# UDC-GAC/pRIblast

Measured on AMD Instinct MI355X. Metric: query RNAs/sec in `ris` step, higher is better.
Workload: dtype f64

## Files before the change

priblast_amd/csrc/capi_search.hip:

```cpp
#include <omp.h>

#include <algorithm>
#include <cmath>
#include <cstdlib>
#include <cstring>
#include <functional>

#include "search_host.hpp"

using namespace prb;

namespace prb {

struct SearchKnobs {
  double budget;
  double chunk_pairs;
  int row_shift;
  bool fused;
  bool front_ahead;
  bool sort_four_keys, sort_two_lengths;
  size_t big_list_bytes;
  int64_t gapped_chunk_hits;
  int first_tier;
  bool wave_hbm, no_resume, front_paired, front, handover;
// ... 129 lines not shown
                h.query + first, h.e_acc + first, h.e_hyb + first, h.e_tot + first};
}
static int bits_for(int64_t max_value) {
  int b = 1;
  while (b < 40 && (int64_t(1) << b) <= max_value) b++;
  return b;
}

static int sort_hits(SubSearch &s, const HitRec *recs, HitSoA out, int64_t n, const SortBounds &sb, uint32_t **perm_out) {
  prb_ctx *ctx = s.ctx;
  SearchWs &w = s.w;
  int rc;
  const size_t N = (size_t)n;
  {
    PackedKeyInfo f;
    f.qmin = sb.qmin;
    f.one_len = sb.eq_len_max > 0;
    f.lmax = f.one_len ? sb.eq_len_max : std::max(sb.max_qlen, sb.max_dblen);
    f.bl = bits_for(f.lmax);
    f.bq = bits_for(sb.max_qlen);
    f.bd = bits_for(sb.nchars);
    const int total = (f.one_len ? 1 : 2) * f.bl + f.bq + f.bd + bits_for(sb.qspan - 1);
    if (total <= 64 && f.lmax <= 65535 && !s.k.sort_four_keys) {
      if ((rc = w.kP.ensure(N * 8)) || (rc = w.kTmp2.ensure(N * 8)) || (rc = w.kE.ensure(N * 8)) || (rc = w.kTmp.ensure(N * 8)) ||
          (rc = w.idxA.ensure(N * 4)) || (rc = w.idxB.ensure(N * 4)) || (rc = w.pending.ensure(16)))
        return rc;
      PRB_HIP(launch_make_packed_keys_recs(recs, n, f, w.kP.as<uint64_t>(), w.kE.as<uint64_t>(), w.idxA.as<uint32_t>(), ctx->stream));
      if ((rc = sort_pairs(ctx->stream, w.sortTmp, w.kP.as<uint64_t>(), w.kTmp2.as<uint64_t>(), w.idxA.as<uint32_t>(),
                           w.idxB.as<uint32_t>(), N, (unsigned)total)))
        return rc;
      PRB_HIP(launch_gather_u64(w.kE.as<uint64_t>(), w.idxB.as<uint32_t>(), w.kTmp.as<uint64_t>(), n, ctx->stream));
      PRB_HIP(hipMemsetAsync(w.pending.p, 0, 4, ctx->stream));
      PRB_HIP(launch_fix_ties(w.kTmp2.as<uint64_t>(), w.kTmp.as<uint64_t>(), w.idxB.as<uint32_t>(), n, recs, w.idxA.as<uint32_t>(),
                              w.pending.as<int32_t>(), ctx->stream));
      int32_t too_long = 0;
      PRB_HIP(hipMemcpyAsync(&too_long, w.pending.p, 4, hipMemcpyDeviceToHost, ctx->stream));
      PRB_HIP(hipStreamSynchronize(ctx->stream));
      if (!too_long) {
        PRB_HIP(launch_gather_recs_to_hits(recs, w.idxA.as<uint32_t>(), out, n, ctx->stream));
        *perm_out = w.idxA.as<uint32_t>();
        return PRB_OK;
      }
    }
  }
  if (s.k.debug_mem) fprintf(stderr, "[mem] sort: the general form (%lld hits)\n", (long long)n);
  if ((rc = w.hitsTmp.ensure(hits_bytes(n)))) return rc;
  const HitSoA in = carve_hits(w.hitsTmp, n);
  PRB_HIP(launch_gather_recs_to_hits(recs, nullptr, in, n, ctx->stream));
  if ((rc = w.kE.ensure(N * 8)) || (rc = w.kL.ensure(N * 4)) || (rc = w.kQ.ensure(N * 4)) || (rc = w.kP.ensure(N * 8)) ||
      (rc = w.kTmp.ensure(N * 8)) || (rc = w.kTmp2.ensure(N * 8)) || (rc = w.idxA.ensure(N * 4)) ||
      (rc = w.idxB.ensure(N * 4)))
    return rc;
  PRB_HIP(launch_make_keys(in, n, w.kE.as<uint64_t>(), w.kL.as<uint32_t>(), w.kQ.as<uint32_t>(), w.kP.as<uint64_t>(),
                           w.idxA.as<uint32_t>(), ctx->stream));
  uint32_t *ia = w.idxA.as<uint32_t>(), *ib = w.idxB.as<uint32_t>();
  auto sort_step = [&](auto *keys, unsigned bits) -> int {
    using K = std::remove_pointer_t<decltype(keys)>;
    if (int r = sort_pairs(ctx->stream, w.sortTmp, keys, w.kTmp2.as<K>(), ia, ib, N, bits)) return r;
// ... 7 lines not shown
  if ((rc = sort_step(w.kTmp.as<uint64_t>(), 64))) return rc;
  PRB_HIP(launch_gather_u64(w.kE.as<uint64_t>(), ia, w.kTmp.as<uint64_t>(), n, ctx->stream));
  if ((rc = sort_step(w.kTmp.as<uint64_t>(), 64))) return rc;
  PRB_HIP(launch_gather_u32(w.kL.as<uint32_t>(), ia, w.kTmp.as<uint32_t>(), n, ctx->stream));
  if ((rc = sort_step(w.kTmp.as<uint32_t>(), 32))) return rc;
  PRB_HIP(launch_gather_u32(w.kQ.as<uint32_t>(), ia, w.kTmp.as<uint32_t>(), n, ctx->stream));
  if ((rc = sort_step(w.kTmp.as<uint32_t>(), 32))) return rc;
  PRB_HIP(launch_gather_u64(w.kP.as<uint64_t>(), ia, w.kTmp.as<uint64_t>(), n, ctx->stream));
  unsigned qbits = 1;
  while ((1 << qbits) < s.qb->nq && qbits < 31) qbits++;
  if ((rc = sort_step(w.kTmp.as<uint64_t>(), 32 + qbits))) return rc;
  PRB_HIP(launch_gather_hits(in, ia, out, n, ctx->stream));
  *perm_out = ia;
  return PRB_OK;
}

struct ToI64 {
  __host__ __device__ int64_t operator()(const int32_t &v) const { return (int64_t)v; }
};
struct MaxOp {
  __host__ __device__ int64_t operator()(const int64_t &a, const int64_t &b) const { return a > b ? a : b; }
};

static int filter_hits(prb_ctx *ctx, SearchWs &w, const HitSoA &h, int64_t n, double thr, int64_t *nsurv) {
  int rc;
  const size_t N = (size_t)n;
  *nsurv = 0;
  if (n == 0) return PRB_OK;
  if ((rc = w.endKey.ensure(N * 8)) || (rc = w.pmax.ensure(N * 8)) || (rc = w.state.ensure(N)) || (rc = w.keep.ensure(N)) ||
      (rc = w.pending.ensure(16)) || (rc = w.surv.ensure(N * 4)) || (rc = w.count.ensure(16)))
    return rc;
  PRB_HIP(launch_filter_init(h, n, thr, w.endKey.as<int64_t>(), w.state.as<uint8_t>(), ctx->stream));
  if ((rc = with_temp(w.scanTmp, "rocprim::inclusive_scan", [&](void *t, size_t &b) {
         return rocprim::inclusive_scan(t, b, w.endKey.as<int64_t>(), w.pmax.as<int64_t>(), N, MaxOp(), ctx->stream);
       })))
    return rc;
  for (int round = 0;; round++) {
    PRB_HIP(hipMemsetAsync(w.pending.p, 0, 4, ctx->stream));
    PRB_HIP(launch_filter_round(h, n, w.pmax.as<int64_t>(), w.state.as<uint8_t>(), w.pending.as<int32_t>(), ctx->stream));
    int32_t pend = 0;
    PRB_HIP(hipMemcpyAsync(&pend, w.pending.p, 4, hipMemcpyDeviceToHost, ctx->stream));
    PRB_HIP(hipStreamSynchronize(ctx->stream));
    if (!pend) break;
    if (round > 100000) {
      set_error("redundancy filter did not converge");
      return PRB_ERR_STATE;
    }
  }
  PRB_HIP(launch_filter_final(h, n, w.pmax.as<int64_t>(), w.state.as<uint8_t>(), w.keep.as<uint8_t>(), ctx->stream));
  return select_flagged(ctx, w, nullptr, w.keep.as<uint8_t>(), w.surv.as<uint32_t>(), N, nsurv);
}

static void mem_note(const char *where, const SearchWs &w) {
  static const bool on = getenv("PRB_DEBUG_MEM") != nullptr;
  if (!on) return;
  size_t free_b = 0, total_b = 0;
  (void)hipMemGetInfo(&free_b, &total_b);
  fprintf(stderr, "[mem] %-18s free %7zu MiB | hitsA %6zu hitsB %6zu hitsC %6zu hitsTmp %6zu MiB\n", where, free_b >> 20, w.hitsA.cap >> 20,
          w.hitsB.cap >> 20, w.hitsC.cap >> 20, w.hitsTmp.cap >> 20);
}

static int grow_keep(prb_ctx *ctx, DevBuf &buf, size_t have, size_t need, size_t spare_limit = SIZE_MAX) {
  int rc;
  if (have > 0 && need > buf.cap) {
    DevBuf bigger;
    if ((rc = need > spare_limit ? PRB_ERR_NOMEM : bigger.ensure(need + need / 2)) && (rc = bigger.ensure(need + need / 6)) &&
        (rc = bigger.ensure(need)))
      return rc;
    PRB_HIP(hipMemcpyAsync(bigger.p, buf.p, have, hipMemcpyDeviceToDevice, ctx->stream));
    PRB_HIP(hipStreamSynchronize(ctx->stream));
    buf.release();
    buf = bigger;
// ... 254 lines not shown
  if (big_list) {
    w.trim_next = true;
    PRB_HIP(hipStreamSynchronize(ctx->stream));
    w.front.release();
    for (DevBuf *b : {&w.hitsA, &w.hitsTmp, &w.row_count, &w.row_off, &w.row_cand, &w.seed_qacc, &w.cands, &w.trace, &w.resumePool,
                      &w.resumePool2, &w.resumePool3, &w.keptU, &w.keptTrace})
      b->release();
    for (DevBuf *b : {&ctx->ra_band, &ctx->ra_vec, &ctx->ra_codes, &ctx->ra_desc}) b->release();
    if ((rc = w.front.init())) return rc;
  }
  mem_note("before the sort", w);
  if ((rc = w.hitsC.ensure(hits_bytes(s.nf)))) return rc;
  HitSoA B = carve_hits(w.hitsC, s.nf);
  uint32_t *perm = nullptr;
  if ((rc = ctx->time_begin())) return rc;
  SortBounds sb1 = s.sb;
  if (s.all_one_pass && s.one_pass_maxlen > 0 && !s.k.sort_two_lengths) sb1.eq_len_max = (int32_t)s.one_pass_maxlen;
  if ((rc = sort_hits(s, w.hitsB.as<HitRec>(), B, s.nf, sb1, &perm))) return rc;
  if ((rc = ctx->time_end("sort", 9))) return rc;
  if (big_list)
    for (DevBuf *b : {&w.hitsB, &w.kE, &w.kL, &w.kQ, &w.kP, &w.kTmp, &w.kTmp2, &w.idxA, &w.idxB, &w.sortTmp}) b->release();
  mem_note("sorted", w);
  if ((rc = ctx->time_begin())) return rc;
  if ((rc = filter_hits(ctx, w, B, s.nf, s.opts.interaction_threshold, &s.nung))) return rc;
  if ((rc = ctx->time_end("filter", 3))) return rc;
  s.hs->counts[1] += s.nung;
  if (s.nung == 0) return PRB_OK;
  if ((rc = w.hitsA.ensure(hits_bytes(s.nung)))) return rc;
  s.U = carve_hits(w.hitsA, s.nung);
  PRB_HIP(launch_gather_hits(B, w.surv.as<uint32_t>(), s.U, s.nung, ctx->stream));
  if ((rc = w.first.ensure((size_t)s.nung))) return rc;
  PRB_HIP(launch_mark_first(s.U.query, s.nung, w.first.as<uint8_t>(), ctx->stream));
  s.first = w.first.as<uint8_t>();
  return PRB_OK;
}

static int emit_ungapped(SubSearch &s) {
  prb_hitset *hs = s.hs;
  const size_t base = hs->hits.size();
  if (int rc = download_hits(s.ctx, s.w, s.U, s.nung, hs->hits)) return rc;
  auto code_base = [](unsigned c) { return c <= 5 ? (int)c - 1 : (int)c - 5; };
  for (size_t i = base; i < hs->hits.size(); i++) {
    prb_hit &h = hs->hits[i];
    const uint8_t *qs = s.qb->enc.data() + s.qb->off[h.query];
    h.bp_offset = (int64_t)hs->bp.size() / 2;
    const int len = (int)(uint16_t)h.q_len;
    for (int j = 0; j < len; j++)
      if (s.ctx->params.bp_pair[code_base(qs[h.q_sp + j])][code_base(s.pg.seqs[h.db_sp + j])] != 0) {
// ... 310 lines not shown
  s.tier_all = w.keptTier.as<uint8_t>();
  s.ntrace_all = w.keptNtrace.as<int32_t>();
  s.trace_all = w.keptTrace.as<uint16_t>();
  return PRB_OK;
}

static int final_sort_filter(SubSearch &s) {
  prb_ctx *ctx = s.ctx;
  SearchWs &w = s.w;
  int rc;
  if (!s.chunked) {
    if ((rc = ctx->time_begin())) return rc;
    if ((rc = compact_below(ctx, w, s.G, s.nung, s.opts.final_threshold, w.cidx, w.hitsB, &s.ngap))) return rc;
    if ((rc = ctx->time_end("filter", 2))) return rc;
  }
  if (s.ngap == 0) return PRB_OK;
  if ((rc = w.hitsC.ensure(hits_bytes(s.ngap)))) return rc;
  HitSoA S = carve_hits(w.hitsC, s.ngap);
  uint32_t *perm = nullptr;
  if ((rc = ctx->time_begin())) return rc;
  if ((rc = sort_hits(s, w.hitsB.as<HitRec>(), S, s.ngap, s.sb, &perm))) return rc;
  if ((rc = ctx->time_end("sort", 9))) return rc;
  if ((rc = ctx->time_begin())) return rc;
  if ((rc = filter_hits(ctx, w, S, s.ngap, s.opts.final_threshold, &s.nfin))) return rc;
  if ((rc = ctx->time_end("filter", 3))) return rc;
  s.hs->counts[2] += s.nfin;
  if (s.nfin == 0) return PRB_OK;
  if ((rc = w.hitsB.ensure(hits_bytes(s.nfin)))) return rc;
  s.F = carve_hits(w.hitsB, s.nfin);
  PRB_HIP(launch_gather_hits(S, w.surv.as<uint32_t>(), s.F, s.nfin, ctx->stream));
  if ((rc = w.subset2.ensure((size_t)s.nfin * 4)) || (rc = w.subset.ensure((size_t)s.nfin * 4))) return rc;
  PRB_HIP(launch_gather_u32(perm, w.surv.as<uint32_t>(), w.subset2.as<uint32_t>(), s.nfin, ctx->stream));
  PRB_HIP(launch_gather_u32(w.cidx.as<uint32_t>(), w.subset2.as<uint32_t>(), w.subset.as<uint32_t>(), s.nfin, ctx->stream));
  return PRB_OK;
}

static int traceback(SubSearch &s) {
  prb_ctx *ctx = s.ctx;
  SearchWs &w = s.w;
  const int64_t nfin = s.nfin;
  const size_t NF = (size_t)nfin;
  int rc;
  if ((rc = w.copy_init())) return rc;
  if (w.copy_pending) {
    PRB_HIP(hipStreamWaitEvent(ctx->stream, w.copy_done, 0));
    w.copy_pending = false;
  }
  if ((rc = ctx->time_begin())) return rc;
// ... 560 lines not shown
```

priblast_amd/csrc/search_host.hpp:

```cpp
#pragma once
#include <atomic>
#include <chrono>
#include <condition_variable>
#include <cstring>
#include <deque>
#include <memory>
#include <mutex>
#include <thread>

#include <rocprim/rocprim.hpp>

#include "../../include/priblast_hip.h"
#include "context.hpp"
#include "db_format.hpp"
#include "hitset.hpp"
#include "output.hpp"
#include "search_kernels.hpp"
#include "seed_dfs.hpp"

namespace prb {

struct SearchConstMem {
  DevBuf ints, bulge;
  SearchConst view{};
// ... 49 lines not shown
        (void)hipStreamDestroy(stream);
        (void)hipEventDestroy(done);
        stream = nullptr;
      }
      for (DevBuf *b : {&cands, &seed_qacc, &pair0, &keyA, &keyB, &valA, &valB, &sortTmp}) b->release();
      pair0_pin.release();
      ahead = false;
    }
  } front;
  hipStream_t copy_stream = nullptr;
  hipEvent_t packed_ready = nullptr, copy_done = nullptr;
  bool copy_pending = false;
  int copy_init() {
    if (copy_stream) return PRB_OK;
    if (hipStreamCreateWithFlags(&copy_stream, hipStreamNonBlocking) != hipSuccess ||
        hipEventCreateWithFlags(&packed_ready, hipEventDisableTiming) != hipSuccess ||
        hipEventCreateWithFlags(&copy_done, hipEventDisableTiming) != hipSuccess) {
      set_error("hipStreamCreate / hipEventCreate failed (result copies)");
      return PRB_ERR_HIP;
    }
    return PRB_OK;
  }
  PinnedBuf pinned, cand_pinned[2], tb_pinned, pin_hits[2], pin_bp[2];
  bool trim_next = false;
  void trim() {
#define X(name, trimmable) \
  if (trimmable && name.cap > ((size_t)256 << 20)) name.release();
    PRB_SEARCH_BUFFERS(X)
#undef X
    trim_next = false;
  }
  void release() {
#define X(name, trimmable) name.release();
    PRB_SEARCH_BUFFERS(X)
#undef X
    front.release();
    if (copy_stream) {
      (void)hipStreamSynchronize(copy_stream);
      (void)hipStreamDestroy(copy_stream);
      (void)hipEventDestroy(packed_ready);
      (void)hipEventDestroy(copy_done);
      copy_stream = nullptr;
    }
    for (PinnedBuf *b : {&pinned, &cand_pinned[0], &cand_pinned[1], &tb_pinned, &pin_hits[0], &pin_hits[1], &pin_bp[0], &pin_bp[1]})
      b->release();
  }
};

inline SearchWs &ws_of(prb_ctx *ctx) {
  if (!ctx->search_ws) ctx->search_ws = new SearchWs();
  return *static_cast<SearchWs *>(ctx->search_ws);
}

struct Drainer {
  struct Job {
    int slot;
    int64_t nhits, nbp_ints;
  };
  std::vector<prb_hit> *hits;
  std::vector<int32_t> *bp;
  std::vector<prb_pair_summary> *pairs = nullptr;
  PinnedBuf *pin_hits, *pin_bp;
  hipEvent_t ev[2] = {nullptr, nullptr};
  std::thread th;
  std::mutex m;
  std::condition_variable cv;
  std::deque<Job> jobs;
// ... 265 lines not shown
```

priblast_amd/csrc/search_kernels.hip:

```cpp
#include "search_kernels.hpp"

#include <cstdlib>

#include "../../include/priblast_hip.h"

#include "search_device.hpp"

namespace prb {

namespace {

constexpr int kBlock = 256;

__device__ __forceinline__ int seq_of(const PageDev &pg, int sp) {
  int lo = 0, hi = pg.nseq - 1;
  while (lo < hi) {
    int m = (lo + hi + 1) >> 1;
    if (pg.start_pos[m] <= sp) lo = m;
    else hi = m - 1;
  }
  return lo;
}

__device__ __forceinline__ double window_acc(const float *acc, const float *cond, int64_t sp, int length, int delta) {
// ... 590 lines not shown
  k_energy[i] = (eb >> 63) ? ~eb : (eb | 0x8000000000000000ull);
  k_len[i] = ((uint32_t)(0xFFFF - US(h.db_len[i])) << 16) | (uint32_t)(0xFFFF - US(h.q_len[i]));
  k_qsp[i] = (uint32_t)h.q_sp[i];
  k_pos[i] = ((uint64_t)(uint32_t)h.query[i] << 32) | (uint32_t)h.db_sp[i];
  idx[i] = (uint32_t)i;
}

__global__ __launch_bounds__(kBlock) void k_make_packed_keys(HitSoA h, int64_t n, PackedKeyInfo f, uint64_t *key,
                                                             uint64_t *k_energy, uint32_t *idx) {
  const int64_t i = (int64_t)blockIdx.x * kBlock + threadIdx.x;
  if (i >= n) return;
  const uint64_t eb = (uint64_t)__double_as_longlong(h.e_tot[i]);
  k_energy[i] = (eb >> 63) ? ~eb : (eb | 0x8000000000000000ull);
  uint64_t k = (uint64_t)(uint32_t)(h.query[i] - f.qmin);
  k = (k << f.bd) | (uint32_t)h.db_sp[i];
  k = (k << f.bq) | (uint32_t)h.q_sp[i];
  k = (k << f.bl) | (uint32_t)(f.lmax - US(h.db_len[i]));
  k = (k << f.bl) | (uint32_t)(f.lmax - US(h.q_len[i]));
  key[i] = k;
  idx[i] = (uint32_t)i;
}

__global__ __launch_bounds__(kBlock) void k_make_packed_keys_recs(const HitRec *__restrict__ h, int64_t n, PackedKeyInfo f,
                                                                  uint64_t *key, uint64_t *k_energy, uint32_t *idx) {
  const int64_t i = (int64_t)blockIdx.x * kBlock + threadIdx.x;
  if (i >= n) return;
  const HitRec r = h[i];
  const uint64_t eb = (uint64_t)__double_as_longlong(r.e_tot);
  k_energy[i] = (eb >> 63) ? ~eb : (eb | 0x8000000000000000ull);
  uint64_t k = (uint64_t)(uint32_t)(r.query - f.qmin);
  k = (k << f.bd) | (uint32_t)r.db_sp;
  k = (k << f.bq) | (uint32_t)r.q_sp;
  k = (k << f.bl) | (uint32_t)(f.lmax - US(r.db_len));
  if (!f.one_len) k = (k << f.bl) | (uint32_t)(f.lmax - US(r.q_len));
  key[i] = k;
  idx[i] = (uint32_t)i;
}

constexpr int kMaxTieRun = 4096;
__device__ __forceinline__ uint64_t order_bits(double v) {
  const uint64_t b = (uint64_t)__double_as_longlong(v);
  return (b >> 63) ? ~b : (b | 0x8000000000000000ull);
}
__global__ __launch_bounds__(kBlock) void k_fix_ties(const uint64_t *__restrict__ key, const uint64_t *__restrict__ e,
                                                     const uint32_t *__restrict__ perm, int64_t n, const HitRec *__restrict__ recs,
                                                     uint32_t *__restrict__ perm_out, int32_t *too_long) {
  const int64_t i = (int64_t)blockIdx.x * kBlock + threadIdx.x;
  if (i >= n) return;
  const uint64_t k = key[i];
  const uint32_t pi = perm[i];
  const bool left = i > 0 && key[i - 1] == k, right = i + 1 < n && key[i + 1] == k;
  if (!left && !right) {
    perm_out[i] = pi;
    return;
  }
  int64_t s = i, t = i + 1;
  while (s > 0 && key[s - 1] == k && i - s <= kMaxTieRun) s--;
  while (t < n && key[t] == k && t - s <= kMaxTieRun) t++;
  if (t - s > kMaxTieRun) {
    *too_long = 1;
    perm_out[i] = pi;
    return;
  }
  const uint64_t ei = e[i];
  const uint64_t hi = order_bits(recs[pi].e_hyb), ai = order_bits(recs[pi].e_acc);
  int rank = 0;
  for (int64_t b = s; b < t; b++) {
    if (b == i) continue;
    const uint64_t eb = e[b];
    bool before = eb < ei;
    if (eb == ei) {
      const uint32_t pb = perm[b];
      const uint64_t hb = order_bits(recs[pb].e_hyb);
      if (hb != hi) {
        before = hb < hi;
      } else {
        const uint64_t ab = order_bits(recs[pb].e_acc);
        before = ab != ai ? ab < ai : pb < pi;
      }
    }
    rank += before ? 1 : 0;
  }
  perm_out[s + rank] = pi;
}

__global__ __launch_bounds__(kBlock) void k_order_keys(const double *__restrict__ v, int64_t n, uint64_t *__restrict__ key) {
  const int64_t i = (int64_t)blockIdx.x * kBlock + threadIdx.x;
  if (i < n) key[i] = order_bits(v[i]);
}

template <class T> __global__ __launch_bounds__(kBlock) void k_gather(const T *src, const uint32_t *idx, T *dst, int64_t n) {
  const int64_t i = (int64_t)blockIdx.x * kBlock + threadIdx.x;
  if (i < n) dst[i] = src[idx[i]];
}

// ... 611 lines not shown
    w.qe[k] = qs + US(h.q_len[g]) - 1;
    w.de[k] = ds + US(h.db_len[g]) - 1;
    w.query[k] = h.query[g];
    w.e[k] = h.e_tot[g];
    w.pmax[k] = pmax[g];
    w.state[k] = state[g];
  }
  __syncthreads();
}
__device__ __forceinline__ Box window_box(const FilterWindow &w, const HitSoA &h, int64_t g) {
  if (g >= w.w0 && g < w.w1) {
    const int k = (int)(g - w.w0);
    return Box{w.qs[k], w.qe[k], w.ds[k], w.de[k], w.query[k], w.e[k]};
  }
  return box_of(h, g);
}
__device__ __forceinline__ int64_t window_pmax(const FilterWindow &w, const int64_t *__restrict__ pmax, int64_t g) {
  return g >= w.w0 && g < w.w1 ? w.pmax[g - w.w0] : pmax[g];
}
__device__ __forceinline__ uint8_t window_state(const FilterWindow &w, const uint8_t *state, int64_t g) {
  return g >= w.w0 && g < w.w1 ? ((const volatile uint8_t *)w.state)[g - w.w0] : ((const volatile uint8_t *)state)[g];
}

__global__ __launch_bounds__(kBlock) void k_filter_round_tile(HitSoA h, int64_t n, const int64_t *__restrict__ pmax, uint8_t *state,
                                                              int32_t *pending) {
  __shared__ FilterWindow w;
  __shared__ int s_progress;
  const int64_t t0 = (int64_t)blockIdx.x * kBlock, i = t0 + threadIdx.x;
  window_load(w, h, n, pmax, state, t0, 0);
  bool mine = i < n && window_state(w, state, i) == kUnknown;
  const Box b = i < n ? window_box(w, h, i) : Box{0, 0, 0, 0, 0, 0.0};
  const int64_t need = pack_end(b.query, b.de);
  for (int iter = 0; iter < 64; iter++) {
    if (threadIdx.x == 0) s_progress = 0;
    __syncthreads();
    if (mine) {
      bool wait = false;
      uint8_t res = kActive;
      for (int64_t a = i - 1; a >= 0; a--) {
        if (window_pmax(w, pmax, a) < need) break;
        const Box c = window_box(w, h, a);
        if (c.query != b.query) break;
        if (contains(c, b) && c.e <= b.e) {
          const uint8_t sa = window_state(w, state, a);
          if (sa == kActive) {
            res = kInactive;
            wait = false;
            break;
          }
          if (sa == kUnknown) wait = true;
        }
      }
      if (!wait) {
        ((volatile uint8_t *)w.state)[i - w.w0] = res;
        state[i] = res;
        mine = false;
        s_progress = 1;
      }
    }
    __syncthreads();
    const int p = s_progress;
    __syncthreads();
    if (!p) break;
  }
  if (mine) *pending = 1;
}

__global__ __launch_bounds__(kBlock) void k_filter_final_tile(HitSoA h, int64_t n, const int64_t *__restrict__ pmax,
                                                              const uint8_t *__restrict__ state, uint8_t *keep) {
  __shared__ FilterWindow w;
  const int64_t t0 = (int64_t)blockIdx.x * kBlock, i = t0 + threadIdx.x;
  window_load(w, h, n, pmax, state, t0, kFilterFwd);
  if (i >= n) return;
  uint8_t k = 0;
  if (window_state(w, state, i) == kActive) {
    k = 1;
    const Box a = window_box(w, h, i);
    for (int64_t j = i + 1; j < n && k; j++) {
      const Box b = window_box(w, h, j);
      if (b.query != a.query || b.ds > a.de) break;
      if (contains(a, b) && a.e > b.e) {
        const int64_t need = pack_end(b.query, b.de);
        bool flagged = false;
        for (int64_t c = i - 1; c >= 0; c--) {
          if (window_pmax(w, pmax, c) < need) break;
          const Box x = window_box(w, h, c);
          if (x.query != b.query) break;
          if (window_state(w, state, c) == kActive && contains(x, b) && x.e <= b.e) {
            flagged = true;
            break;
          }
        }
        if (!flagged) k = 0;
      }
    }
  }
  keep[i] = k;
}

inline dim3 grid_for(int64_t n) { return dim3((unsigned)((n + kBlock - 1) / kBlock)); }

}

hipError_t launch_sa_seq(const PageDev &pg, int32_t *sa_seq, hipStream_t s) {
  if (pg.nchars <= 0) return hipSuccess;
  hipLaunchKernelGGL(k_sa_seq, grid_for(pg.nchars), dim3(kBlock), 0, s, pg, sa_seq);
  return hipGetLastError();
}
hipError_t launch_seed_qacc(const CandDev *cands, int32_t ncand, int64_t nq_entries, const QBatchDev &qb, int delta, double *qacc,
                            hipStream_t s) {
  if (nq_entries <= 0) return hipSuccess;
  hipLaunchKernelGGL(k_seed_qacc, grid_for(nq_entries), dim3(kBlock), 0, s, cands, ncand, nq_entries, qb, delta, qacc);
  return hipGetLastError();
}
hipError_t launch_row_keys(const CandDev *cands, int32_t ncand, int64_t nrows, const PageDev &pg, int qmin, int shift, int dbits,
                           bool wide, int32_t *row_cand, void *key, uint32_t *val, hipStream_t s) {
  if (nrows <= 0) return hipSuccess;
  if (wide)
    hipLaunchKernelGGL(k_row_key<uint64_t>, grid_for(nrows), dim3(kBlock), 0, s, cands, ncand, nrows, pg, qmin, shift, dbits, row_cand,
                       (uint64_t *)key, val);
// ... 54 lines not shown
}
hipError_t launch_ungapped(HitSoA hits, int64_t n, const QBatchDev &qb, const PageDev &pg, const SearchConst &sc, ExtOpts o,
                           int max_query_len, hipStream_t s) {
  if (n <= 0) return hipSuccess;
  int qcap = (max_query_len + 1 + 3) & ~3;
  if (qcap > 7168) qcap = 7168;
  const int64_t per_block = (int64_t)kBlock * kUngappedPer;
  hipLaunchKernelGGL(k_ungapped, dim3((unsigned)((n + per_block - 1) / per_block)), dim3(kBlock), (size_t)qcap * 9, s, hits, n,
                     qb, pg, sc, o, qcap);
  return hipGetLastError();
}
hipError_t launch_make_keys(const HitSoA &hits, int64_t n, uint64_t *k_energy, uint32_t *k_len, uint32_t *k_qsp,
                            uint64_t *k_pos, uint32_t *idx, hipStream_t s) {
  if (n <= 0) return hipSuccess;
  hipLaunchKernelGGL(k_make_keys, grid_for(n), dim3(kBlock), 0, s, hits, n, k_energy, k_len, k_qsp, k_pos, idx);
  return hipGetLastError();
}
hipError_t launch_make_packed_keys(const HitSoA &hits, int64_t n, const PackedKeyInfo &f, uint64_t *key, uint64_t *k_energy,
                                   uint32_t *idx, hipStream_t s) {
  if (n <= 0) return hipSuccess;
  hipLaunchKernelGGL(k_make_packed_keys, grid_for(n), dim3(kBlock), 0, s, hits, n, f, key, k_energy, idx);
  return hipGetLastError();
}
hipError_t launch_fix_ties(const uint64_t *key_sorted, const uint64_t *e_sorted, const uint32_t *perm, int64_t n, const HitRec *recs,
                           uint32_t *perm_out, int32_t *too_long, hipStream_t s) {
  if (n <= 0) return hipSuccess;
  hipLaunchKernelGGL(k_fix_ties, grid_for(n), dim3(kBlock), 0, s, key_sorted, e_sorted, perm, n, recs, perm_out, too_long);
  return hipGetLastError();
}
hipError_t launch_order_keys(const double *v, int64_t n, uint64_t *key, hipStream_t s) {
  if (n <= 0) return hipSuccess;
  hipLaunchKernelGGL(k_order_keys, grid_for(n), dim3(kBlock), 0, s, v, n, key);
  return hipGetLastError();
}
hipError_t launch_gather_u64(const uint64_t *src, const uint32_t *idx, uint64_t *dst, int64_t n, hipStream_t s) {
  if (n <= 0) return hipSuccess;
  hipLaunchKernelGGL(k_gather<uint64_t>, grid_for(n), dim3(kBlock), 0, s, src, idx, dst, n);
  return hipGetLastError();
}
hipError_t launch_gather_u32(const uint32_t *src, const uint32_t *idx, uint32_t *dst, int64_t n, hipStream_t s) {
  if (n <= 0) return hipSuccess;
  hipLaunchKernelGGL(k_gather<uint32_t>, grid_for(n), dim3(kBlock), 0, s, src, idx, dst, n);
  return hipGetLastError();
}
namespace {
__global__ __launch_bounds__(256) void k_iota_u32(uint32_t *dst, int64_t n) {
  const int64_t i = (int64_t)blockIdx.x * 256 + threadIdx.x;
  if (i < n) dst[i] = (uint32_t)i;
}
__global__ __launch_bounds__(256) void k_gather_rows(const uint4 *__restrict__ src, const uint32_t *__restrict__ idx, uint4 *dst, int64_t n,
// ... 30 lines not shown
                     static_cast<uint4 *>(dst), n, words);
  return hipGetLastError();
}
hipError_t launch_gather_u8(const uint8_t *src, const uint32_t *idx, uint8_t *dst, int64_t n, hipStream_t s) {
  if (n <= 0) return hipSuccess;
  hipLaunchKernelGGL(k_gather<uint8_t>, grid_for(n), dim3(kBlock), 0, s, src, idx, dst, n);
  return hipGetLastError();
}
hipError_t launch_gather_hits(const HitSoA &src, const uint32_t *idx, HitSoA dst, int64_t n, hipStream_t s) {
  if (n <= 0) return hipSuccess;
  hipLaunchKernelGGL(k_gather_hits, grid_for(n), dim3(kBlock), 0, s, src, idx, dst, n);
  return hipGetLastError();
}
hipError_t launch_gather_hits_to_recs(const HitSoA &src, const uint32_t *idx, HitRec *dst, int64_t n, hipStream_t s) {
  if (n <= 0) return hipSuccess;
  hipLaunchKernelGGL(k_gather_hits_to_recs, grid_for(n), dim3(kBlock), 0, s, src, idx, dst, n);
  return hipGetLastError();
}
hipError_t launch_gather_recs_to_hits(const HitRec *src, const uint32_t *idx, HitSoA dst, int64_t n, hipStream_t s) {
  if (n <= 0) return hipSuccess;
  hipLaunchKernelGGL(k_gather_recs_to_hits, grid_for(n), dim3(kBlock), 0, s, src, idx, dst, n);
  return hipGetLastError();
}
hipError_t launch_make_packed_keys_recs(const HitRec *hits, int64_t n, const PackedKeyInfo &f, uint64_t *key, uint64_t *k_energy,
                                        uint32_t *idx, hipStream_t s) {
  if (n <= 0) return hipSuccess;
  hipLaunchKernelGGL(k_make_packed_keys_recs, grid_for(n), dim3(kBlock), 0, s, hits, n, f, key, k_energy, idx);
  return hipGetLastError();
}
hipError_t launch_pack_hits(const HitSoA &src, int64_t n, const int32_t *bp_count, const int64_t *bp_off, int64_t bp_base,
                            void *out, hipStream_t s) {
  if (n <= 0) return hipSuccess;
  hipLaunchKernelGGL(k_pack_hits, grid_for(n), dim3(kBlock), 0, s, src, n, bp_count, bp_off, bp_base, static_cast<prb_hit *>(out));
  return hipGetLastError();
}
hipError_t launch_pair_heads(const int32_t *query, const int32_t *db_id, int64_t n, uint8_t *head, hipStream_t s) {
  if (n <= 0) return hipSuccess;
  hipLaunchKernelGGL(k_pair_heads, grid_for(n), dim3(kBlock), 0, s, query, db_id, n, head);
  return hipGetLastError();
}
hipError_t launch_pair_fold(const HitSoA &h, int64_t n, const uint32_t *start, int64_t npairs, const int32_t *ends, void *out,
                            hipStream_t s) {
  if (npairs <= 0 || n <= 0) return hipSuccess;
  hipLaunchKernelGGL(k_pair_fold, grid_for(npairs), dim3(kBlock), 0, s, h, n, start, npairs, ends, static_cast<prb_pair_summary *>(out));
  return hipGetLastError();
}
template <class R>
static hipError_t launch_top_merge_of(const void *rec, int64_t nrec, int32_t q0, int32_t q1, int32_t page, int32_t n, void *tab,
                                      int32_t *fill, hipStream_t s) {
  if (nrec <= 0 || q1 <= q0) return hipSuccess;
// ... 59 lines not shown
                            hipStream_t s) {
  if (n <= 0) return hipSuccess;
  hipLaunchKernelGGL(k_prof_rows, grid_for(n), dim3(kBlock), 0, s, t, idx, n, hits, targets, static_cast<prb_profile_pos *>(rows));
  return hipGetLastError();
}
hipError_t launch_flag_not_above(const double *e_tot, int64_t n, double thr, uint8_t *keep, hipStream_t s) {
  if (n <= 0) return hipSuccess;
  hipLaunchKernelGGL(k_flag_not_above, grid_for(n), dim3(kBlock), 0, s, e_tot, n, thr, keep);
  return hipGetLastError();
}
hipError_t launch_mark_first(const int32_t *query, int64_t n, uint8_t *first, hipStream_t s) {
  if (n <= 0) return hipSuccess;
  hipLaunchKernelGGL(k_mark_first, grid_for(n), dim3(kBlock), 0, s, query, n, first);
  return hipGetLastError();
}
hipError_t launch_filter_init(const HitSoA &h, int64_t n, double thr, int64_t *end_key, uint8_t *state, hipStream_t s) {
  if (n <= 0) return hipSuccess;
  hipLaunchKernelGGL(k_filter_init, grid_for(n), dim3(kBlock), 0, s, h, n, thr, end_key, state);
  return hipGetLastError();
}
hipError_t launch_filter_round(const HitSoA &h, int64_t n, const int64_t *pmax, uint8_t *state, int32_t *pending,
                               hipStream_t s) {
  if (n <= 0) return hipSuccess;
  const bool tiles = !(getenv("PRB_FILTER_TILES") && atoi(getenv("PRB_FILTER_TILES")) == 0);
  if (tiles) hipLaunchKernelGGL(k_filter_round_tile, grid_for(n), dim3(kBlock), 0, s, h, n, pmax, state, pending);
  else hipLaunchKernelGGL(k_filter_round, grid_for(n), dim3(kBlock), 0, s, h, n, pmax, state, pending);
  return hipGetLastError();
}
hipError_t launch_filter_final(const HitSoA &h, int64_t n, const int64_t *pmax, const uint8_t *state, uint8_t *keep,
                               hipStream_t s) {
  if (n <= 0) return hipSuccess;
  const bool tiles = !(getenv("PRB_FILTER_TILES") && atoi(getenv("PRB_FILTER_TILES")) == 0);
  if (tiles) hipLaunchKernelGGL(k_filter_final_tile, grid_for(n), dim3(kBlock), 0, s, h, n, pmax, state, keep);
  else hipLaunchKernelGGL(k_filter_final, grid_for(n), dim3(kBlock), 0, s, h, n, pmax, state, keep);
  return hipGetLastError();
}
}
```

priblast_amd/csrc/search_kernels.hpp:

```cpp
#pragma once
#include <hip/hip_runtime.h>

#include <cstdint>

namespace prb {

struct SearchTab {
  static constexpr int kStack = 0;
  static constexpr int kInternal = kStack + 49;
  static constexpr int kMismatchI = kInternal + 31;
  static constexpr int kInt11 = kMismatchI + 175;
  static constexpr int kInt21 = kInt11 + 1600;
  static constexpr int kInt22 = kInt21 + 8000;
  static constexpr int kDangle5 = kInt22 + 40000;
  static constexpr int kDangle3 = kDangle5 + 40;
  static constexpr int kBulge = kDangle3 + 40;
  static constexpr int kTau = kBulge + 31;
  static constexpr int kZero = kTau + 8;
  static constexpr int kCount = kZero + 1;
};

struct SearchConst {
  const int32_t *tab;
  const int32_t *stack37;
// ... 118 lines not shown
hipError_t launch_prof_rows(const ProfTab &t, const uint32_t *idx, int64_t n, const int64_t *hits, const int32_t *targets, void *rows,
                            hipStream_t s);
hipError_t launch_gather_u8(const uint8_t *src, const uint32_t *idx, uint8_t *dst, int64_t n, hipStream_t s);
hipError_t launch_iota_u32(uint32_t *dst, int64_t n, hipStream_t s);
hipError_t launch_flag_marked(const uint8_t *marks, const uint32_t *list, int64_t n, uint8_t mask, uint8_t *flags, hipStream_t s);
hipError_t launch_gather_rows(const void *src, const uint32_t *idx, void *dst, int64_t n, int row_bytes, hipStream_t s);
hipError_t launch_gather_hits(const HitSoA &src, const uint32_t *idx, HitSoA dst, int64_t n, hipStream_t s);
struct alignas(16) HitRec {
  int32_t q_sp, db_sp, q_len, db_len, db_id, db_id_start, query, pad0;
  double e_acc, e_hyb, e_tot;
  int64_t pad1;
};
static_assert(sizeof(HitRec) == 64, "one cache line half, two per 128-byte line");
constexpr int64_t kMaxFusedCands = 1 << 20, kMaxFusedEntries = 1 << 12;
hipError_t launch_pair_keys(const CandDev *cands, const int64_t *pair0, int32_t ncand, int64_t npairs, const PageDev &pg, int qmin,
                            int shift, int dbits, bool wide, void *key, uint64_t *val, hipStream_t s);
constexpr int kFusePairs = 2048, kSliceRecBytes = 48;
inline int64_t fused_slices(int64_t npairs) { return (npairs + kFusePairs - 1) / kFusePairs; }
hipError_t launch_seed_extend(const CandDev *cands, const uint64_t *vals, int64_t npairs, const QBatchDev &qb, const PageDev &pg,
                              const SearchConst &sc, ExtOpts o, const double *qacc, double thr, int max_query_len, void *slices,
                              int32_t *slice_count, uint64_t *nseed, hipStream_t s);
hipError_t launch_collect_slices(const void *slices, const int32_t *slice_count, const int64_t *slice_off, int64_t nslices, HitRec *out,
                                 hipStream_t s);
hipError_t launch_fix_ties(const uint64_t *key_sorted, const uint64_t *e_sorted, const uint32_t *perm, int64_t n, const HitRec *recs,
                           uint32_t *perm_out, int32_t *too_long, hipStream_t s);
hipError_t launch_gather_hits_to_recs(const HitSoA &src, const uint32_t *idx, HitRec *dst, int64_t n, hipStream_t s);
hipError_t launch_gather_recs_to_hits(const HitRec *src, const uint32_t *idx, HitSoA dst, int64_t n, hipStream_t s);
hipError_t launch_make_packed_keys_recs(const HitRec *hits, int64_t n, const PackedKeyInfo &f, uint64_t *key, uint64_t *k_energy,
                                        uint32_t *idx, hipStream_t s);
hipError_t launch_flag_not_above(const double *e_tot, int64_t n, double thr, uint8_t *keep, hipStream_t s);
hipError_t launch_mark_first(const int32_t *query, int64_t n, uint8_t *first, hipStream_t s);
hipError_t launch_filter_init(const HitSoA &h, int64_t n, double thr, int64_t *db_end_key, uint8_t *state, hipStream_t s);
hipError_t launch_filter_round(const HitSoA &h, int64_t n, const int64_t *pmax, uint8_t *state, int32_t *pending,
                               hipStream_t s);
hipError_t launch_filter_final(const HitSoA &h, int64_t n, const int64_t *pmax, const uint8_t *state, uint8_t *keep,
                               hipStream_t s);
constexpr size_t kGapWaveLdsBytes = 64 * 1024;
struct GapScratch {
  uint8_t *base;
  size_t bytes_per_thread;
  int32_t cap_rec, cap_diag;
  int32_t nthreads;
};
size_t gapped_wave_scratch_bytes(int cap_diag, int cap_rec);
struct GapResume {
  int32_t *slot;
  uint8_t *pool;
  uint32_t *count;
  int32_t cap;
};
size_t gapped_resume_bytes(int tier);
hipError_t launch_gapped_lds(const HitSoA &in, HitSoA out, int64_t n, const uint32_t *subset, const QBatchDev &qb,
                             const PageDev &pg, const SearchConst &sc, ExtOpts o, int mode, int tier, uint8_t *overflow,
                             uint8_t *tier_out, const uint8_t *first_flag, int32_t *bp_count, uint16_t *trace,
                             const int64_t *bp_off, int32_t *bp_out, unsigned long long *next_work ,
                             const GapResume &rin, const GapResume &rout, hipStream_t s, int handover = 0 ,
                             double *acc_scratch = nullptr );
size_t gapped_acc_scratch_bytes();
constexpr int kTraceCap = 32;
// ... 33 lines not shown
```

Measured before the change: 7.577.

## Fuse filter rounds and final pass into a worklist-driven tile kernel

Replaces the iterative redundancy filter, which relaunched a full-grid round kernel until convergence and then ran a separate final kernel, with a single tile kernel. Each launch only processes tiles still holding unresolved hits, using a compacted worklist ping-ponged inside the reused endKey buffer, and writes keep flags directly. It also drops the separate energy-key array and its gather from the packed sort path, recomputing energy order bits from records in the tie fixer. Host readbacks now go to a pinned word instead of a stack variable. The cost is extra redundant window resolution for the preceding region in each block and some scattered record reads during tie fixing.

```diff
diff --git a/priblast_amd/csrc/capi_search.hip b/priblast_amd/csrc/capi_search.hip
--- a/priblast_amd/csrc/capi_search.hip
+++ b/priblast_amd/csrc/capi_search.hip
@@ -175,18 +175,17 @@
     f.bd = bits_for(sb.nchars);
     const int total = (f.one_len ? 1 : 2) * f.bl + f.bq + f.bd + bits_for(sb.qspan - 1);
     if (total <= 64 && f.lmax <= 65535 && !s.k.sort_four_keys) {
-      if ((rc = w.kP.ensure(N * 8)) || (rc = w.kTmp2.ensure(N * 8)) || (rc = w.kE.ensure(N * 8)) || (rc = w.kTmp.ensure(N * 8)) ||
-          (rc = w.idxA.ensure(N * 4)) || (rc = w.idxB.ensure(N * 4)) || (rc = w.pending.ensure(16)))
+      if ((rc = w.kP.ensure(N * 8)) || (rc = w.kTmp2.ensure(N * 8)) || (rc = w.idxA.ensure(N * 4)) || (rc = w.idxB.ensure(N * 4)) ||
+          (rc = w.pending.ensure(16)) || (rc = w.word.ensure(16)))
         return rc;
-      PRB_HIP(launch_make_packed_keys_recs(recs, n, f, w.kP.as<uint64_t>(), w.kE.as<uint64_t>(), w.idxA.as<uint32_t>(), ctx->stream));
+      PRB_HIP(launch_make_packed_keys_recs(recs, n, f, w.kP.as<uint64_t>(), w.idxA.as<uint32_t>(), ctx->stream));
       if ((rc = sort_pairs(ctx->stream, w.sortTmp, w.kP.as<uint64_t>(), w.kTmp2.as<uint64_t>(), w.idxA.as<uint32_t>(),
                            w.idxB.as<uint32_t>(), N, (unsigned)total)))
         return rc;
-      PRB_HIP(launch_gather_u64(w.kE.as<uint64_t>(), w.idxB.as<uint32_t>(), w.kTmp.as<uint64_t>(), n, ctx->stream));
       PRB_HIP(hipMemsetAsync(w.pending.p, 0, 4, ctx->stream));
-      PRB_HIP(launch_fix_ties(w.kTmp2.as<uint64_t>(), w.kTmp.as<uint64_t>(), w.idxB.as<uint32_t>(), n, recs, w.idxA.as<uint32_t>(),
-                              w.pending.as<int32_t>(), ctx->stream));
-      int32_t too_long = 0;
+      PRB_HIP(launch_fix_ties(w.kTmp2.as<uint64_t>(), w.idxB.as<uint32_t>(), n, recs, w.idxA.as<uint32_t>(), w.pending.as<int32_t>(),
+                              ctx->stream));
+      int32_t &too_long = *static_cast<int32_t *>(w.word.p);
       PRB_HIP(hipMemcpyAsync(&too_long, w.pending.p, 4, hipMemcpyDeviceToHost, ctx->stream));
       PRB_HIP(hipStreamSynchronize(ctx->stream));
       if (!too_long) {
@@ -240,32 +239,57 @@
   __host__ __device__ int64_t operator()(const int64_t &a, const int64_t &b) const { return a > b ? a : b; }
 };
 
-static int filter_hits(prb_ctx *ctx, SearchWs &w, const HitSoA &h, int64_t n, double thr, int64_t *nsurv) {
+static int filter_hits(prb_ctx *ctx, SearchWs &w, const HitSoA &h, int64_t n, double thr, int64_t *nsurv, int64_t *launches) {
   int rc;
   const size_t N = (size_t)n;
   *nsurv = 0;
+  *launches = 0;
   if (n == 0) return PRB_OK;
   if ((rc = w.endKey.ensure(N * 8)) || (rc = w.pmax.ensure(N * 8)) || (rc = w.state.ensure(N)) || (rc = w.keep.ensure(N)) ||
-      (rc = w.pending.ensure(16)) || (rc = w.surv.ensure(N * 4)) || (rc = w.count.ensure(16)))
+      (rc = w.pending.ensure(16)) || (rc = w.surv.ensure(N * 4)) || (rc = w.count.ensure(16)) || (rc = w.word.ensure(16)))
     return rc;
   PRB_HIP(launch_filter_init(h, n, thr, w.endKey.as<int64_t>(), w.state.as<uint8_t>(), ctx->stream));
   if ((rc = with_temp(w.scanTmp, "rocprim::inclusive_scan", [&](void *t, size_t &b) {
          return rocprim::inclusive_scan(t, b, w.endKey.as<int64_t>(), w.pmax.as<int64_t>(), N, MaxOp(), ctx->stream);
        })))
     return rc;
-  for (int round = 0;; round++) {
-    PRB_HIP(hipMemsetAsync(w.pending.p, 0, 4, ctx->stream));
-    PRB_HIP(launch_filter_round(h, n, w.pmax.as<int64_t>(), w.state.as<uint8_t>(), w.pending.as<int32_t>(), ctx->stream));
-    int32_t pend = 0;
-    PRB_HIP(hipMemcpyAsync(&pend, w.pending.p, 4, hipMemcpyDeviceToHost, ctx->stream));
-    PRB_HIP(hipStreamSynchronize(ctx->stream));
-    if (!pend) break;
-    if (round > 100000) {
-      set_error("redundancy filter did not converge");
-      return PRB_ERR_STATE;
+  const bool tiles = !env_off(getenv("PRB_FILTER_TILES"));
+  int32_t &pend = *static_cast<int32_t *>(w.word.p);
+  int64_t rounds = 0;
+  if (tiles) {
+    const int64_t ntiles = filter_tiles(n);
+    uint32_t *lists[2] = {w.endKey.as<uint32_t>(), w.endKey.as<uint32_t>() + ntiles};
+    const uint32_t *todo = nullptr;
+    for (int64_t m = ntiles; m > 0; rounds++) {
+      if (rounds > 100000) {
+        set_error("redundancy filter did not converge");
+        return PRB_ERR_STATE;
+      }
+      uint32_t *left = lists[rounds & 1];
+      PRB_HIP(hipMemsetAsync(w.pending.p, 0, 4, ctx->stream));
+      PRB_HIP(launch_filter_tile(h, n, w.pmax.as<int64_t>(), w.state.as<uint8_t>(), w.keep.as<uint8_t>(), todo, m, left,
+                                 w.pending.as<int32_t>(), ctx->stream));
+      PRB_HIP(hipMemcpyAsync(&pend, w.pending.p, 4, hipMemcpyDeviceToHost, ctx->stream));
+      PRB_HIP(hipStreamSynchronize(ctx->stream));
+      m = pend;
+      todo = left;
     }
-  }
-  PRB_HIP(launch_filter_final(h, n, w.pmax.as<int64_t>(), w.state.as<uint8_t>(), w.keep.as<uint8_t>(), ctx->stream));
+  } else {
+    for (;; rounds++) {
+      PRB_HIP(hipMemsetAsync(w.pending.p, 0, 4, ctx->stream));
+      PRB_HIP(launch_filter_round(h, n, w.pmax.as<int64_t>(), w.state.as<uint8_t>(), w.pending.as<int32_t>(), ctx->stream));
+      PRB_HIP(hipMemcpyAsync(&pend, w.pending.p, 4, hipMemcpyDeviceToHost, ctx->stream));
+      PRB_HIP(hipStreamSynchronize(ctx->stream));
+      if (!pend) break;
+      if (rounds > 100000) {
+        set_error("redundancy filter did not converge");
+        return PRB_ERR_STATE;
+      }
+    }
+    PRB_HIP(launch_filter_final(h, n, w.pmax.as<int64_t>(), w.state.as<uint8_t>(), w.keep.as<uint8_t>(), ctx->stream));
+    rounds += 2;
+  }
+  *launches = 3 + rounds;
   return select_flagged(ctx, w, nullptr, w.keep.as<uint8_t>(), w.surv.as<uint32_t>(), N, nsurv);
 }
 
@@ -566,8 +590,9 @@
     for (DevBuf *b : {&w.hitsB, &w.kE, &w.kL, &w.kQ, &w.kP, &w.kTmp, &w.kTmp2, &w.idxA, &w.idxB, &w.sortTmp}) b->release();
   mem_note("sorted", w);
   if ((rc = ctx->time_begin())) return rc;
-  if ((rc = filter_hits(ctx, w, B, s.nf, s.opts.interaction_threshold, &s.nung))) return rc;
-  if ((rc = ctx->time_end("filter", 3))) return rc;
+  int64_t launches = 0;
+  if ((rc = filter_hits(ctx, w, B, s.nf, s.opts.interaction_threshold, &s.nung, &launches))) return rc;
+  if ((rc = ctx->time_end("filter", launches))) return rc;
   s.hs->counts[1] += s.nung;
   if (s.nung == 0) return PRB_OK;
   if ((rc = w.hitsA.ensure(hits_bytes(s.nung)))) return rc;
@@ -924,8 +949,9 @@
   if ((rc = sort_hits(s, w.hitsB.as<HitRec>(), S, s.ngap, s.sb, &perm))) return rc;
   if ((rc = ctx->time_end("sort", 9))) return rc;
   if ((rc = ctx->time_begin())) return rc;
-  if ((rc = filter_hits(ctx, w, S, s.ngap, s.opts.final_threshold, &s.nfin))) return rc;
-  if ((rc = ctx->time_end("filter", 3))) return rc;
+  int64_t launches = 0;
+  if ((rc = filter_hits(ctx, w, S, s.ngap, s.opts.final_threshold, &s.nfin, &launches))) return rc;
+  if ((rc = ctx->time_end("filter", launches))) return rc;
   s.hs->counts[2] += s.nfin;
   if (s.nfin == 0) return PRB_OK;
   if ((rc = w.hitsB.ensure(hits_bytes(s.nfin)))) return rc;
diff --git a/priblast_amd/csrc/search_host.hpp b/priblast_amd/csrc/search_host.hpp
--- a/priblast_amd/csrc/search_host.hpp
+++ b/priblast_amd/csrc/search_host.hpp
@@ -95,6 +95,7 @@
     return PRB_OK;
   }
   PinnedBuf pinned, cand_pinned[2], tb_pinned, pin_hits[2], pin_bp[2];
+  PinnedBuf word;
   bool trim_next = false;
   void trim() {
 #define X(name, trimmable) \
@@ -115,7 +116,7 @@
       (void)hipEventDestroy(copy_done);
       copy_stream = nullptr;
     }
-    for (PinnedBuf *b : {&pinned, &cand_pinned[0], &cand_pinned[1], &tb_pinned, &pin_hits[0], &pin_hits[1], &pin_bp[0], &pin_bp[1]})
+    for (PinnedBuf *b : {&pinned, &cand_pinned[0], &cand_pinned[1], &tb_pinned, &pin_hits[0], &pin_hits[1], &pin_bp[0], &pin_bp[1], &word})
       b->release();
   }
 };
diff --git a/priblast_amd/csrc/search_kernels.hip b/priblast_amd/csrc/search_kernels.hip
--- a/priblast_amd/csrc/search_kernels.hip
+++ b/priblast_amd/csrc/search_kernels.hip
@@ -636,12 +636,10 @@
 }
 
 __global__ __launch_bounds__(kBlock) void k_make_packed_keys_recs(const HitRec *__restrict__ h, int64_t n, PackedKeyInfo f,
-                                                                  uint64_t *key, uint64_t *k_energy, uint32_t *idx) {
+                                                                  uint64_t *key, uint32_t *idx) {
   const int64_t i = (int64_t)blockIdx.x * kBlock + threadIdx.x;
   if (i >= n) return;
   const HitRec r = h[i];
-  const uint64_t eb = (uint64_t)__double_as_longlong(r.e_tot);
-  k_energy[i] = (eb >> 63) ? ~eb : (eb | 0x8000000000000000ull);
   uint64_t k = (uint64_t)(uint32_t)(r.query - f.qmin);
   k = (k << f.bd) | (uint32_t)r.db_sp;
   k = (k << f.bq) | (uint32_t)r.q_sp;
@@ -656,9 +654,8 @@
   const uint64_t b = (uint64_t)__double_as_longlong(v);
   return (b >> 63) ? ~b : (b | 0x8000000000000000ull);
 }
-__global__ __launch_bounds__(kBlock) void k_fix_ties(const uint64_t *__restrict__ key, const uint64_t *__restrict__ e,
-                                                     const uint32_t *__restrict__ perm, int64_t n, const HitRec *__restrict__ recs,
-                                                     uint32_t *__restrict__ perm_out, int32_t *too_long) {
+__global__ __launch_bounds__(kBlock) void k_fix_ties(const uint64_t *__restrict__ key, const uint32_t *__restrict__ perm, int64_t n,
+                                                     const HitRec *__restrict__ recs, uint32_t *__restrict__ perm_out, int32_t *too_long) {
   const int64_t i = (int64_t)blockIdx.x * kBlock + threadIdx.x;
   if (i >= n) return;
   const uint64_t k = key[i];
@@ -676,15 +673,15 @@
     perm_out[i] = pi;
     return;
   }
-  const uint64_t ei = e[i];
+  const uint64_t ei = order_bits(recs[pi].e_tot);
   const uint64_t hi = order_bits(recs[pi].e_hyb), ai = order_bits(recs[pi].e_acc);
   int rank = 0;
   for (int64_t b = s; b < t; b++) {
     if (b == i) continue;
-    const uint64_t eb = e[b];
+    const uint32_t pb = perm[b];
+    const uint64_t eb = order_bits(recs[pb].e_tot);
     bool before = eb < ei;
     if (eb == ei) {
-      const uint32_t pb = perm[b];
       const uint64_t hb = order_bits(recs[pb].e_hyb);
       if (hb != hi) {
         before = hb < hi;
@@ -1342,80 +1339,99 @@
   return g >= w.w0 && g < w.w1 ? ((const volatile uint8_t *)w.state)[g - w.w0] : ((const volatile uint8_t *)state)[g];
 }
 
-__global__ __launch_bounds__(kBlock) void k_filter_round_tile(HitSoA h, int64_t n, const int64_t *__restrict__ pmax, uint8_t *state,
-                                                              int32_t *pending) {
+__device__ __forceinline__ bool window_resolve(const FilterWindow &w, const HitSoA &h, const int64_t *__restrict__ pmax, const uint8_t *state,
+                                               int64_t g, const Box &b, uint8_t *res) {
+  const int64_t need = pack_end(b.query, b.de);
+  bool wait = false;
+  for (int64_t a = g - 1; a >= 0; a--) {
+    if (window_pmax(w, pmax, a) < need) break;
+    const Box c = window_box(w, h, a);
+    if (c.query != b.query) break;
+    if (contains(c, b) && c.e <= b.e) {
+      const uint8_t sa = window_state(w, state, a);
+      if (sa == kActive) {
+        *res = kInactive;
+        return true;
+      }
+      if (sa == kUnknown) wait = true;
+    }
+  }
+  *res = kActive;
+  return !wait;
+}
+
+__global__ __launch_bounds__(kBlock) void k_filter_tile(HitSoA h, int64_t n, const int64_t *__restrict__ pmax, uint8_t *state, uint8_t *keep,
+                                                        const uint32_t *__restrict__ tiles_in, uint32_t *__restrict__ tiles_out,
+                                                        int32_t *ntiles_out) {
   __shared__ FilterWindow w;
-  __shared__ int s_progress;
-  const int64_t t0 = (int64_t)blockIdx.x * kBlock, i = t0 + threadIdx.x;
-  window_load(w, h, n, pmax, state, t0, 0);
-  bool mine = i < n && window_state(w, state, i) == kUnknown;
-  const Box b = i < n ? window_box(w, h, i) : Box{0, 0, 0, 0, 0, 0.0};
-  const int64_t need = pack_end(b.query, b.de);
+  __shared__ int s_progress, s_left;
+  const int64_t tile = tiles_in ? (int64_t)tiles_in[blockIdx.x] : (int64_t)blockIdx.x;
+  const int64_t t0 = tile * kBlock, i = t0 + threadIdx.x;
+  if (threadIdx.x == 0) s_left = 0;
+  window_load(w, h, n, pmax, state, t0, kFilterFwd);
+  const int64_t w0 = w.w0;
+  const int64_t g1 = w0 + threadIdx.x;
+  bool mine0 = i < n && w.state[i - w0] == kUnknown;
+  bool mine1 = g1 < t0 && w.state[g1 - w0] == kUnknown;
+  const Box b0 = i < n ? window_box(w, h, i) : Box{0, 0, 0, 0, 0, 0.0};
+  const Box b1 = g1 < t0 ? window_box(w, h, g1) : Box{0, 0, 0, 0, 0, 0.0};
   for (int iter = 0; iter < 64; iter++) {
     if (threadIdx.x == 0) s_progress = 0;
     __syncthreads();
-    if (mine) {
-      bool wait = false;
-      uint8_t res = kActive;
-      for (int64_t a = i - 1; a >= 0; a--) {
-        if (window_pmax(w, pmax, a) < need) break;
-        const Box c = window_box(w, h, a);
-        if (c.query != b.query) break;
-        if (contains(c, b) && c.e <= b.e) {
-          const uint8_t sa = window_state(w, state, a);
-          if (sa == kActive) {
-            res = kInactive;
-            wait = false;
-            break;
-          }
-          if (sa == kUnknown) wait = true;
-        }
-      }
-      if (!wait) {
-        ((volatile uint8_t *)w.state)[i - w.w0] = res;
-        state[i] = res;
-        mine = false;
-        s_progress = 1;
-      }
+    uint8_t res;
+    if (mine0 && window_resolve(w, h, pmax, state, i, b0, &res)) {
+      ((volatile uint8_t *)w.state)[i - w0] = res;
+      state[i] = res;
+      mine0 = false;
+      s_progress = 1;
+    }
+    if (mine1 && window_resolve(w, h, pmax, state, g1, b1, &res)) {
+      ((volatile uint8_t *)w.state)[g1 - w0] = res;
+      mine1 = false;
+      s_progress = 1;
     }
     __syncthreads();
     const int p = s_progress;
     __syncthreads();
     if (!p) break;
   }
-  if (mine) *pending = 1;
-}
-
-__global__ __launch_bounds__(kBlock) void k_filter_final_tile(HitSoA h, int64_t n, const int64_t *__restrict__ pmax,
-                                                              const uint8_t *__restrict__ state, uint8_t *keep) {
-  __shared__ FilterWindow w;
-  const int64_t t0 = (int64_t)blockIdx.x * kBlock, i = t0 + threadIdx.x;
-  window_load(w, h, n, pmax, state, t0, kFilterFwd);
-  if (i >= n) return;
-  uint8_t k = 0;
-  if (window_state(w, state, i) == kActive) {
-    k = 1;
-    const Box a = window_box(w, h, i);
-    for (int64_t j = i + 1; j < n && k; j++) {
-      const Box b = window_box(w, h, j);
-      if (b.query != a.query || b.ds > a.de) break;
-      if (contains(a, b) && a.e > b.e) {
-        const int64_t need = pack_end(b.query, b.de);
-        bool flagged = false;
-        for (int64_t c = i - 1; c >= 0; c--) {
-          if (window_pmax(w, pmax, c) < need) break;
-          const Box x = window_box(w, h, c);
-          if (x.query != b.query) break;
-          if (window_state(w, state, c) == kActive && contains(x, b) && x.e <= b.e) {
-            flagged = true;
-            break;
+  bool open = mine0;
+  if (i < n && !mine0) {
+    uint8_t k = 0;
+    if (window_state(w, state, i) == kActive) {
+      k = 1;
+      for (int64_t j = i + 1; j < n && k; j++) {
+        const Box b = window_box(w, h, j);
+        if (b.query != b0.query || b.ds > b0.de) break;
+        if (contains(b0, b) && b0.e > b.e) {
+          const int64_t need = pack_end(b.query, b.de);
+          bool flagged = false, maybe = false;
+          for (int64_t c = i - 1; c >= 0; c--) {
+            if (window_pmax(w, pmax, c) < need) break;
+            const Box x = window_box(w, h, c);
+            if (x.query != b.query) break;
+            if (contains(x, b) && x.e <= b.e) {
+              const uint8_t sc = window_state(w, state, c);
+              if (sc == kActive) {
+                flagged = true;
+                break;
+              }
+              if (sc == kUnknown) maybe = true;
+            }
+          }
+          if (!flagged) {
+            if (maybe) open = true;
+            else k = 0;
           }
         }
-        if (!flagged) k = 0;
       }
-    }
-  }
-  keep[i] = k;
+      if (k == 0) open = false;
+    }
+    if (!open) keep[i] = k;
+  }
+  if (open) s_left = 1;
+  __syncthreads();
+  if (threadIdx.x == 0 && s_left) tiles_out[atomicAdd(ntiles_out, 1)] = (uint32_t)tile;
 }
 
 inline dim3 grid_for(int64_t n) { return dim3((unsigned)((n + kBlock - 1) / kBlock)); }
@@ -1516,10 +1532,10 @@
   hipLaunchKernelGGL(k_make_packed_keys, grid_for(n), dim3(kBlock), 0, s, hits, n, f, key, k_energy, idx);
   return hipGetLastError();
 }
-hipError_t launch_fix_ties(const uint64_t *key_sorted, const uint64_t *e_sorted, const uint32_t *perm, int64_t n, const HitRec *recs,
-                           uint32_t *perm_out, int32_t *too_long, hipStream_t s) {
-  if (n <= 0) return hipSuccess;
-  hipLaunchKernelGGL(k_fix_ties, grid_for(n), dim3(kBlock), 0, s, key_sorted, e_sorted, perm, n, recs, perm_out, too_long);
+hipError_t launch_fix_ties(const uint64_t *key_sorted, const uint32_t *perm, int64_t n, const HitRec *recs, uint32_t *perm_out,
+                           int32_t *too_long, hipStream_t s) {
+  if (n <= 0) return hipSuccess;
+  hipLaunchKernelGGL(k_fix_ties, grid_for(n), dim3(kBlock), 0, s, key_sorted, perm, n, recs, perm_out, too_long);
   return hipGetLastError();
 }
 hipError_t launch_order_keys(const double *v, int64_t n, uint64_t *key, hipStream_t s) {
@@ -1596,10 +1612,10 @@
   hipLaunchKernelGGL(k_gather_recs_to_hits, grid_for(n), dim3(kBlock), 0, s, src, idx, dst, n);
   return hipGetLastError();
 }
-hipError_t launch_make_packed_keys_recs(const HitRec *hits, int64_t n, const PackedKeyInfo &f, uint64_t *key, uint64_t *k_energy,
-                                        uint32_t *idx, hipStream_t s) {
-  if (n <= 0) return hipSuccess;
-  hipLaunchKernelGGL(k_make_packed_keys_recs, grid_for(n), dim3(kBlock), 0, s, hits, n, f, key, k_energy, idx);
+hipError_t launch_make_packed_keys_recs(const HitRec *hits, int64_t n, const PackedKeyInfo &f, uint64_t *key, uint32_t *idx,
+                                        hipStream_t s) {
+  if (n <= 0) return hipSuccess;
+  hipLaunchKernelGGL(k_make_packed_keys_recs, grid_for(n), dim3(kBlock), 0, s, hits, n, f, key, idx);
   return hipGetLastError();
 }
 hipError_t launch_pack_hits(const HitSoA &src, int64_t n, const int32_t *bp_count, const int64_t *bp_off, int64_t bp_base,
@@ -1705,17 +1721,19 @@
 hipError_t launch_filter_round(const HitSoA &h, int64_t n, const int64_t *pmax, uint8_t *state, int32_t *pending,
                                hipStream_t s) {
   if (n <= 0) return hipSuccess;
-  const bool tiles = !(getenv("PRB_FILTER_TILES") && atoi(getenv("PRB_FILTER_TILES")) == 0);
-  if (tiles) hipLaunchKernelGGL(k_filter_round_tile, grid_for(n), dim3(kBlock), 0, s, h, n, pmax, state, pending);
-  else hipLaunchKernelGGL(k_filter_round, grid_for(n), dim3(kBlock), 0, s, h, n, pmax, state, pending);
+  hipLaunchKernelGGL(k_filter_round, grid_for(n), dim3(kBlock), 0, s, h, n, pmax, state, pending);
   return hipGetLastError();
 }
 hipError_t launch_filter_final(const HitSoA &h, int64_t n, const int64_t *pmax, const uint8_t *state, uint8_t *keep,
                                hipStream_t s) {
   if (n <= 0) return hipSuccess;
-  const bool tiles = !(getenv("PRB_FILTER_TILES") && atoi(getenv("PRB_FILTER_TILES")) == 0);
-  if (tiles) hipLaunchKernelGGL(k_filter_final_tile, grid_for(n), dim3(kBlock), 0, s, h, n, pmax, state, keep);
-  else hipLaunchKernelGGL(k_filter_final, grid_for(n), dim3(kBlock), 0, s, h, n, pmax, state, keep);
-  return hipGetLastError();
-}
-}
+  hipLaunchKernelGGL(k_filter_final, grid_for(n), dim3(kBlock), 0, s, h, n, pmax, state, keep);
+  return hipGetLastError();
+}
+hipError_t launch_filter_tile(const HitSoA &h, int64_t n, const int64_t *pmax, uint8_t *state, uint8_t *keep, const uint32_t *tiles_in,
+                              int64_t ntiles, uint32_t *tiles_out, int32_t *ntiles_out, hipStream_t s) {
+  if (n <= 0 || ntiles <= 0) return hipSuccess;
+  hipLaunchKernelGGL(k_filter_tile, dim3((unsigned)ntiles), dim3(kBlock), 0, s, h, n, pmax, state, keep, tiles_in, tiles_out, ntiles_out);
+  return hipGetLastError();
+}
+}
diff --git a/priblast_amd/csrc/search_kernels.hpp b/priblast_amd/csrc/search_kernels.hpp
--- a/priblast_amd/csrc/search_kernels.hpp
+++ b/priblast_amd/csrc/search_kernels.hpp
@@ -164,12 +164,12 @@
                               int32_t *slice_count, uint64_t *nseed, hipStream_t s);
 hipError_t launch_collect_slices(const void *slices, const int32_t *slice_count, const int64_t *slice_off, int64_t nslices, HitRec *out,
                                  hipStream_t s);
-hipError_t launch_fix_ties(const uint64_t *key_sorted, const uint64_t *e_sorted, const uint32_t *perm, int64_t n, const HitRec *recs,
-                           uint32_t *perm_out, int32_t *too_long, hipStream_t s);
+hipError_t launch_fix_ties(const uint64_t *key_sorted, const uint32_t *perm, int64_t n, const HitRec *recs, uint32_t *perm_out,
+                           int32_t *too_long, hipStream_t s);
 hipError_t launch_gather_hits_to_recs(const HitSoA &src, const uint32_t *idx, HitRec *dst, int64_t n, hipStream_t s);
 hipError_t launch_gather_recs_to_hits(const HitRec *src, const uint32_t *idx, HitSoA dst, int64_t n, hipStream_t s);
-hipError_t launch_make_packed_keys_recs(const HitRec *hits, int64_t n, const PackedKeyInfo &f, uint64_t *key, uint64_t *k_energy,
-                                        uint32_t *idx, hipStream_t s);
+hipError_t launch_make_packed_keys_recs(const HitRec *hits, int64_t n, const PackedKeyInfo &f, uint64_t *key, uint32_t *idx,
+                                        hipStream_t s);
 hipError_t launch_flag_not_above(const double *e_tot, int64_t n, double thr, uint8_t *keep, hipStream_t s);
 hipError_t launch_mark_first(const int32_t *query, int64_t n, uint8_t *first, hipStream_t s);
 hipError_t launch_filter_init(const HitSoA &h, int64_t n, double thr, int64_t *db_end_key, uint8_t *state, hipStream_t s);
@@ -177,6 +177,10 @@
                                hipStream_t s);
 hipError_t launch_filter_final(const HitSoA &h, int64_t n, const int64_t *pmax, const uint8_t *state, uint8_t *keep,
                                hipStream_t s);
+constexpr int kFilterTile = 256;
+inline int64_t filter_tiles(int64_t n) { return (n + kFilterTile - 1) / kFilterTile; }
+hipError_t launch_filter_tile(const HitSoA &h, int64_t n, const int64_t *pmax, uint8_t *state, uint8_t *keep, const uint32_t *tiles_in,
+                              int64_t ntiles, uint32_t *tiles_out, int32_t *ntiles_out, hipStream_t s);
 constexpr size_t kGapWaveLdsBytes = 64 * 1024;
 struct GapScratch {
   uint8_t *base;
```

Result: no change. 7.523 (-0.7%).
